# ashual/scene_generation

Hardware: AMD Instinct MI355X
Metric: images/sec G+D step, 128x128 <=8-obj scene graphs (higher is better)
Workload: dtype f32

## Files before the change

### scene_generation_amd/csrc/igemm_core.h

```cpp
#pragma once
#include <type_traits>
#include "common.h"
#include <stdlib.h>
#include <array>
#include <map>
#include <mutex>

typedef float f32x16 __attribute__((ext_vector_type(16)));


namespace sgk {
struct Gather {
  const float* src1; const float* src2;
  int C1, C2;
  int SH, SW;
  int LH, LW;
  int ushift;
  int PH, PW;
  int stride, sshift, pad, reflect;
  int bcast2;
  int pstep, ph0, pw0;
};

struct KEntry { unsigned choff; unsigned tapsel; };
// ... 3 lines not shown
extern thread_local double t_alg_bytes;
extern std::mutex g_tab_mu;
extern std::map<TabKey, TabEntry> g_tabs;
extern size_t g_tab_bytes;

int kn0_run(int KS, const float* A, int M, int K, const Gather& g, int NB, const float* bias, float* out, int Mtot, int act,
            float slope, double flops, void* ktab_ws, size_t ws_avail, hipStream_t s);
int kn1_run(int KS, const float* A, int M, int K, const Gather& g, int NB, const float* bias, float* out, int Mtot, int act,
            float slope, double flops, void* ktab_ws, size_t ws_avail, unsigned variant_stride, hipStream_t s);
int kn_sparse_run(int KS, const float* W, int M, int K, const Gather& g, int NB, const float* bias, float* out, int act,
                  float slope, const Sparse& sp, void* ws, hipStream_t s);
int kn_parity_run(int KS, const float* W, int Rdim, int B, int m0, int M, const Gather& g, int NB, const float* bias,
                  float* out, int Mtot, int act, float slope, double flops, void* ws, size_t ws_bytes, hipStream_t s);
int nk_run(int KS, const float* A, int M, int Mtot, const Gather& g, int NB, float* out, void* ws, size_t ws_bytes,
           double flops, hipStream_t s, const Sparse* sp, float* gb = nullptr, bool* gb_done = nullptr);
int skinny_vec(int align, int ld, int K);
int skinny_gemm(const float* a, int lda, int av, const float* b, int ldb, int bv, float* c, const float* bias,
                float* rowsum, int M, int N, int K, int act, float slope, hipStream_t s);
int skinny_gemm_gather(const float* obj, const float* pred, const int64_t* edges, int T, int Do, int Dp, const float* w, float* c,
                       const float* bias, int N, int act, float slope, hipStream_t s);
inline bool skinny_shape(int M, int N) {
  return (long)sg_cdiv(M, 32) * sg_cdiv(N, 32) <= (long)sg_opt(SG_OPT_LINEAR_SKINNY);
}
}

namespace {
using namespace sgk;
thread_local unsigned t_variant_stride = 0;

#ifdef SG_TIMELINE
__device__ unsigned long long* g_sg_tl = nullptr;
__device__ unsigned g_sg_tl_cap = 0;
#define SG_TL_STAMP(slot)                                                                       \
  do {                                                                                          \
    if (tl_on) tl_rec[slot] = __builtin_amdgcn_s_memtime();                                     \
  } while (0)
#else
#define SG_TL_STAMP(slot) do { } while (0)
#endif

#ifndef SG_NSUB
#define SG_NSUB 1
#endif
constexpr int BK = 16;

#ifndef SG_PIPE_DEFAULT
#define SG_PIPE_DEFAULT 2
#endif
template <int BM_, int BN_, int WGM_, int NSUB_, int PIPE_ = SG_PIPE_DEFAULT, int KFOLD_ = 0, int TS_ = (PIPE_ != 0 ? 1 : 0)>
struct TileCfg {
  static constexpr int BM = BM_, BN = BN_, WGM = WGM_, WGN = 4 / WGM_, NSUB = NSUB_, BKT = BK * NSUB_, PIPE = PIPE_;
  static constexpr int KFOLD = KFOLD_, TAILSPLIT = TS_;
  static_assert(TS_ == 0 || PIPE_ != 0, "tail split: pipelined loop only");
  static_assert(KFOLD_ == 0 || (PIPE_ != 0 && KFOLD_ % (BK * NSUB_) == 0), "KFOLD: whole k-tiles of the pipelined loop");
  static constexpr int WM = BM / WGM, WN = BN / WGN;
  static constexpr int TM = WM / 32, TN = WN / 32;
  static constexpr int LDA = BM + 4, LDB = BN + 4;
};

constexpr int LDK = BK + 4;



#ifndef SG_BUFLOAD
#define SG_BUFLOAD 1
#endif
constexpr int TAP_INVALID = SG_BUFLOAD ? (1 << 29) : -1;
#if SG_BUFLOAD
__device__ __forceinline__ __amdgpu_buffer_rsrc_t sg_rsrc(const float* p) {
  return __builtin_amdgcn_make_buffer_rsrc(const_cast<float*>(p), 0, 0x80000000u, 0x00020000);
}
__device__ __forceinline__ float sg_bufload(__amdgpu_buffer_rsrc_t r, unsigned elem) {
  return __builtin_bit_cast(float, __builtin_amdgcn_raw_buffer_load_b32(r, (int)(elem << 2), 0, 0));
}
__device__ __forceinline__ float4 sg_bufload4(__amdgpu_buffer_rsrc_t r, unsigned elem) {
  const auto v = __builtin_amdgcn_raw_buffer_load_b128(r, (int)(elem << 2), 0, 0);
  static_assert(sizeof(v) == 16, "raw_buffer_load_b128 must return 16 bytes");
  float4 f;
  __builtin_memcpy(&f, &v, 16);
  return f;
}
#endif
typedef unsigned int sg_u32x4 __attribute__((ext_vector_type(4)));
constexpr unsigned ELEM_INVALID = 1u << 29;
constexpr double SG_MAX_ELEMS = SG_BUFLOAD ? 536870912.0 : 2147483647.0;


template <int BX, bool VEC, bool MASK = true>
struct LoadKContig {
  const float* base; int ld; int X;
  static constexpr int LDS_INTS = 0;
  static constexpr int PASSES = BX >= 64 ? BX / 64 : 1;
  struct Stage { float r[PASSES * 4]; unsigned ok; };
  int x0_, xr_, kq_;
  unsigned voff_[PASSES];
  __device__ __forceinline__ void init(int x0, int tid, int*, int, int) {
    x0_ = x0; xr_ = tid >> 2; kq_ = (tid & 3) * 4;
#pragma unroll
    for (int p = 0; p < PASSES; ++p) {
      const int xl = xr_ + p * 64;
      const int x = x0_ + xl;
      const bool xok = (BX % 64 == 0 || xl < BX) && x < X;
      voff_[p] = xok ? ((unsigned)x * (unsigned)ld + (unsigned)kq_) * 4u : 0x80000000u;
    }
  }
  __device__ __forceinline__ void set_batch(int b, int stride, int) { base += (size_t)b * (size_t)stride; }
  __device__ __forceinline__ void prefetch(Stage&, int) const {}
  __device__ __forceinline__ void load(Stage& st, int k0, int kend) const {
    st.ok = 0;
#if SG_BUFLOAD
    if (VEC && (!MASK || k0 + BK <= kend)) {
      const __amdgpu_buffer_rsrc_t rs = sg_rsrc(base);
      const int so = __builtin_amdgcn_readfirstlane(k0 * 4);
#pragma unroll
      for (int p = 0; p < PASSES; ++p) {
        const auto v = __builtin_amdgcn_raw_buffer_load_b128(rs, (int)voff_[p], so, 0);
        __builtin_memcpy(&st.r[p * 4], &v, 16);
      }
      return;
    }
#endif
#pragma unroll
    for (int p = 0; p < PASSES; ++p) {
      const int xl = xr_ + p * 64;
      const int x = x0_ + xl, k = k0 + kq_;
      const bool xok = (BX % 64 == 0 || xl < BX) && x < X;
      const unsigned row = (unsigned)(xok ? x : 0) * (unsigned)ld;
      if (VEC && !MASK) {
        const float4 v = *reinterpret_cast<const float4*>(base + (unsigned)x * (unsigned)ld + k);
        st.r[p * 4 + 0] = v.x; st.r[p * 4 + 1] = v.y; st.r[p * 4 + 2] = v.z; st.r[p * 4 + 3] = v.w;
      } else if (VEC) {
        const bool ok = xok && k < kend;
#if SG_BUFLOAD
        const float4 v = sg_bufload4(sg_rsrc(base), ok ? row + (unsigned)k : ELEM_INVALID);
#else
        const float4 v = *reinterpret_cast<const float4*>(base + row + (ok ? k : 0));
        st.ok |= ok ? (15u << (p * 4)) : 0u;
#endif
        st.r[p * 4 + 0] = v.x; st.r[p * 4 + 1] = v.y; st.r[p * 4 + 2] = v.z; st.r[p * 4 + 3] = v.w;
      } else {
#pragma unroll
        for (int i = 0; i < 4; ++i) {
          const bool ok = xok && k + i < kend;
#if SG_BUFLOAD
          st.r[p * 4 + i] = sg_bufload(sg_rsrc(base), ok ? row + (unsigned)(k + i) : ELEM_INVALID);
#else
          st.r[p * 4 + i] = base[row + (ok ? k + i : 0)];
          st.ok |= ok ? (1u << (p * 4 + i)) : 0u;
#endif
        }
      }
    }
  }
  __device__ __forceinline__ void store(const Stage& st, float* T) const {
#pragma unroll
    for (int p = 0; p < PASSES; ++p) {
      const int xl = xr_ + p * 64;
      const bool in_tile = BX % 64 == 0 || xl < BX;
      if (in_tile && (SG_BUFLOAD || (VEC && !MASK))) {
        *reinterpret_cast<float4*>(T + xl * LDK + kq_) = make_float4(st.r[p * 4], st.r[p * 4 + 1], st.r[p * 4 + 2], st.r[p * 4 + 3]);
      } else if (in_tile) {
        float4 v;
        v.x = ((st.ok >> (p * 4 + 0)) & 1u) ? st.r[p * 4 + 0] : 0.f;
        v.y = ((st.ok >> (p * 4 + 1)) & 1u) ? st.r[p * 4 + 1] : 0.f;
        v.z = ((st.ok >> (p * 4 + 2)) & 1u) ? st.r[p * 4 + 2] : 0.f;
        v.w = ((st.ok >> (p * 4 + 3)) & 1u) ? st.r[p * 4 + 3] : 0.f;
// ... 90 lines not shown
  }
}


__global__ void build_ktab_kernel(KEntry* tab, int K, int Kpad, int KS2, int C1, int C2, unsigned shw, int bcast2,
                                  int tail_valid, unsigned variant_stride) {
  const int k = blockIdx.x * blockDim.x + threadIdx.x;
  if (k >= Kpad) return;
  KEntry e;
  if (k < K) {
    const int c = k / KS2, t = k - c * KS2;
    const bool second = C2 > 0 && c >= C1;
    const unsigned cc = (unsigned)(second ? c - C1 : c);
    e.choff = ((second && bcast2) ? cc : cc * shw) + (unsigned)t * variant_stride;
    e.tapsel = (unsigned)t | (second ? 256u : 0u);
  } else {
    e.choff = 0u; e.tapsel = tail_valid ? 0u : (unsigned)KS2;
  }
  tab[k] = e;
}

template <class Build>
const void* cached_table(TabKey key, size_t bytes, hipStream_t s, Build build) {
  int dev = 0;
  hipGetDevice(&dev);
  key[11] = dev;
  std::lock_guard<std::mutex> lk(g_tab_mu);
  auto it = g_tabs.find(key);
  if (it == g_tabs.end()) {
    TabEntry e{nullptr, bytes, nullptr, s};
    if (hipMalloc(&e.dev, bytes) != hipSuccess) return nullptr;
    hipEventCreateWithFlags(&e.ready, hipEventDisableTiming);
    build(e.dev);
    hipEventRecord(e.ready, s);
    g_tab_bytes += bytes;
    it = g_tabs.emplace(key, e).first;
  } else if (it->second.stream != s) {
    hipStreamCaptureStatus cs = hipStreamCaptureStatusNone;
    if (hipStreamIsCapturing(s, &cs) != hipSuccess || cs == hipStreamCaptureStatusNone) hipStreamWaitEvent(s, it->second.ready, 0);
  }
  return it->second.dev;
}

template <int BN, int KS, int MODE, bool TWO, bool MASK = true>
struct LoadGatherKN {
  Gather g; int Npix; const KEntry* ktab;
  static constexpr int KS2 = KS * KS;
  static constexpr int LDS_INTS = (KS2 + 1) * BN;
  static constexpr int ROWS = BN * BK / 256;
  static constexpr bool BUF = SG_BUFLOAD && MASK;
  struct Stage { float r[ROWS]; unsigned ok; KEntry e[ROWS]; };
  unsigned img1_, img2_, img2b_;
  int nl_, kr_;
  const int* tab_;
  __device__ __forceinline__ void set_batch(int b, int stride, int limit) { ktab += (size_t)b * (size_t)stride; Npix = limit; }
  __device__ __forceinline__ void init(int n0, int tid, int* tab, int, int) {
    nl_ = tid % BN;
    const int grp = tid / BN;
    kr_ = __builtin_amdgcn_readfirstlane(grp * ROWS);
    const int n = n0 + nl_;
    const bool okn = n < Npix;
    const int nn = okn ? n : 0;
    const int phw = g.PH * g.PW;
    const int img = nn / phw;
    const int pix = nn - img * phw;
    const int pi = pix / g.PW;
    const int ph = pi * g.pstep + g.ph0, pw = (pix - pi * g.PW) * g.pstep + g.pw0;
    int ah, aw;
    if (MODE == 0) { ah = ph * g.stride - g.pad; aw = pw * g.stride - g.pad; }
    else { ah = ph + g.pad; aw = pw + g.pad; }
    const unsigned shw = (unsigned)(g.SH * g.SW);
    img1_ = (unsigned)img * (unsigned)g.C1 * shw;
    img2_ = g.bcast2 ? (unsigned)img * (unsigned)g.C2 : (unsigned)img * (unsigned)g.C2 * shw;
    constexpr int G = 256 / BN;
    for (int t = grp; t <= KS2; t += G) {
      const int kh = t / KS, kw = t - kh * KS;
      int v = (okn && t < KS2) ? tap_offset<MODE>(g, ah, aw, kh, kw) : -1;
      if (BUF && v < 0) v = TAP_INVALID;
      tab[t * BN + nl_] = v;
    }
    tab_ = tab + nl_;
  }
  __device__ __forceinline__ void prefetch(Stage& st, int k0) const {
    const KEntry* e = ktab + (k0 + kr_);
#pragma unroll
    for (int i = 0; i < ROWS; ++i) st.e[i] = e[i];
  }
  __device__ __forceinline__ void load(Stage& st, int k0, int kend) const {
#if SG_BUFLOAD
    if (BUF) {
      const __amdgpu_buffer_rsrc_t r1 = sg_rsrc(g.src1);
#pragma unroll
      for (int i = 0; i < ROWS; ++i) {
        const unsigned choff = st.e[i].choff, ts = st.e[i].tapsel;
        const unsigned tp = (unsigned)tab_[(ts & 255u) * BN];
        if (TWO) {
          const bool second = (ts & 256u) != 0u;
          const unsigned t2 = (second && g.bcast2) ? (tp >= (unsigned)TAP_INVALID ? tp : 0u) : tp;
          st.r[i] = sg_bufload(second ? sg_rsrc(g.src2) : r1, (second ? img2_ : img1_) + choff + t2);
        } else {
          st.r[i] = sg_bufload(r1, img1_ + choff + tp);
        }
      }
      return;
    }
#endif
    st.ok = 0;
#pragma unroll
    for (int i = 0; i < ROWS; ++i) {
      const unsigned choff = st.e[i].choff, ts = st.e[i].tapsel;
      const int tp = tab_[(ts & 255u) * BN];
      const bool ok = !MASK || tp >= 0;
      if (TWO) {
        const bool second = (ts & 256u) != 0u;
        const float* base = second ? g.src2 : g.src1;
        const unsigned off = (second ? img2_ : img1_) + choff + ((second && g.bcast2) ? 0u : (unsigned)tp);
        st.r[i] = base[ok ? off : 0u];
      } else {
        st.r[i] = g.src1[ok ? img1_ + choff + (unsigned)tp : 0u];
      }
      st.ok |= ok ? (1u << i) : 0u;
    }
  }
  __device__ __forceinline__ void store(const Stage& st, float* T) const {
    if (BUF) store_krun<ROWS, false>(T, nl_, kr_, st.r, 0u);
    else store_krun<ROWS, MASK>(T, nl_, kr_, st.r, st.ok);
  }
};

struct FixedTaps { int lg; unsigned tapcode; };
template <int BN, int MODE>
struct LoadFixedKN {
  Gather g; int Npix; int KS; int lg; unsigned tapcode;
  int dedup;
  FastDiv dphw, dpw;
  static constexpr int LDS_INTS = 0;
  static constexpr int ROWS = BN * BK / 256;
  struct Stage { float r[ROWS]; };
  int nl_, kr_;
  unsigned voff_[ROWS];
  unsigned shw4_;
  __device__ __forceinline__ void set_batch(int, int, int) {}
  __device__ __forceinline__ void init(int n0, int tid, int*, int, int) {
    nl_ = tid % BN;
    kr_ = __builtin_amdgcn_readfirstlane((tid / BN) * ROWS);
    const int n = n0 + nl_;
    const bool okn = n < Npix;
    const int nn = okn ? n : 0;
    const int phw = g.PH * g.PW;
    const int img = (int)dphw.div((unsigned)nn);
    const int pix = nn - img * phw;
    const int pi = (int)dpw.div((unsigned)pix);
    const int ph = pi * g.pstep + g.ph0, pw = (pix - pi * g.PW) * g.pstep + g.pw0;
    int ah, aw;
    if (MODE == 0) { ah = ph * g.stride - g.pad; aw = pw * g.stride - g.pad; }
    else { ah = ph + g.pad; aw = pw + g.pad; }
    const unsigned shw = (unsigned)(g.SH * g.SW);
    shw4_ = shw * 4u;
    const unsigned img1 = (unsigned)img * (unsigned)g.C1 * shw;
    const int nt = 1 << lg;
    auto tap_voff = [&](int ti) -> unsigned {
      const int t = lg == 4 ? ti : (int)((tapcode >> (4 * ti)) & 15u);
      const int kh = KS == 4 ? (t >> 2) : (KS == 3 ? ((t * 11) >> 5) : (KS == 1 ? 0 : t / KS)), kw = t - kh * KS;
      const int v = okn ? tap_offset<MODE>(g, ah, aw, kh, kw) : -1;
      return v < 0 ? 0x80000000u : (img1 + (unsigned)v) * 4u;
    };
    if (lg <= 2 && dedup) {
      unsigned o[4];
      o[0] = tap_voff(0);
// ... 772 lines not shown
      for (int i = 0; i < TM; ++i) a[i] = *reinterpret_cast<const float4*>(A_ + i * 32 * LDK);
#pragma unroll
      for (int j = 0; j < TN; ++j) b[j] = *reinterpret_cast<const float4*>(B_ + j * 32 * LDK);
    };
    auto mma = [&](const float4 (&a)[TM], const float4 (&b)[TN]) {
#pragma unroll
      for (int e = 0; e < 4; ++e)
#pragma unroll
        for (int i = 0; i < TM; ++i)
#pragma unroll
          for (int j = 0; j < TN; ++j) {
            const float av = e == 0 ? a[i].x : (e == 1 ? a[i].y : (e == 2 ? a[i].z : a[i].w));
            const float bv = e == 0 ? b[j].x : (e == 1 ? b[j].y : (e == 2 ? b[j].z : b[j].w));
            acc[i][j] = __builtin_amdgcn_mfma_f32_32x32x2f32(av, bv, acc[i][j], 0, 0, 0);
          }
    };
    if (kbeg + BKT < kend) {
#pragma unroll
      for (int u = 0; u < NSUB; ++u) { al.load(sa[u], kbeg + BKT + u * BK, kend); bl.load(sb[u], kbeg + BKT + u * BK, kend); }
#pragma unroll
      for (int u = 0; u < NSUB; ++u) { al.prefetch(sa[u], kbeg + 2 * BKT + u * BK); bl.prefetch(sb[u], kbeg + 2 * BKT + u * BK); }
    }
    read_frag(0, 0, fa[0], fb[0]);
    if (AL::LDS_INTS > 0 || BL::LDS_INTS > 0) __syncthreads();
    constexpr bool FOLD = CFG::KFOLD > 0;
    f32x16 acc2[FOLD ? TM : 1][FOLD ? TN : 1];
    if constexpr (FOLD) {
#pragma unroll
      for (int i = 0; i < TM; ++i)
#pragma unroll
        for (int j = 0; j < TN; ++j)
#pragma unroll
          for (int r = 0; r < 16; ++r) acc2[i][j][r] = 0.f;
    }
    for (int k0 = kbeg; k0 < kend; k0 += BKT) {
      const bool more1 = k0 + BKT < kend, more2 = k0 + 2 * BKT < kend;
      if constexpr (FOLD) {
        if (k0 > kbeg && ((k0 - kbeg) % CFG::KFOLD) == 0) {
#pragma unroll
          for (int i = 0; i < TM; ++i)
#pragma unroll
            for (int j = 0; j < TN; ++j)
#pragma unroll
              for (int r = 0; r < 16; ++r) { acc2[i][j][r] += acc[i][j][r]; acc[i][j][r] = 0.f; }
        }
      }
      constexpr bool INTER = CFG::PIPE == 2 && 2 * NSUB <= 4;
      auto stage_next = [&]() {
        if (more2) {
#pragma unroll
          for (int u = 0; u < NSUB; ++u) { al.load(sa[u], k0 + 2 * BKT + u * BK, kend); bl.load(sb[u], k0 + 2 * BKT + u * BK, kend); }
#pragma unroll
          for (int u = 0; u < NSUB; ++u) { al.prefetch(sa[u], k0 + 3 * BKT + u * BK); bl.prefetch(sb[u], k0 + 3 * BKT + u * BK); }
        }
      };
      if (!INTER) {
        if (more1) {
#pragma unroll
          for (int u = 0; u < NSUB; ++u) { al.store(sa[u], As[buf ^ 1] + u * BM * LDK); bl.store(sb[u], Bs[buf ^ 1] + u * BN * LDK); }
        }
        stage_next();
      }
#pragma unroll
      for (int p = 0; p < P - 1; ++p) {
        read_frag(buf, p + 1, fa[(p + 1) & 1], fb[(p + 1) & 1]);
        __builtin_amdgcn_sched_barrier(0);
        if (INTER && p == 0) {
#pragma unroll
          for (int e = 0; e < 4; ++e) {
#pragma unroll
            for (int i = 0; i < TM; ++i)
#pragma unroll
              for (int j = 0; j < TN; ++j) {
                const float av = e == 0 ? fa[0][i].x : (e == 1 ? fa[0][i].y : (e == 2 ? fa[0][i].z : fa[0][i].w));
                const float bv = e == 0 ? fb[0][j].x : (e == 1 ? fb[0][j].y : (e == 2 ? fb[0][j].z : fb[0][j].w));
                acc[i][j] = __builtin_amdgcn_mfma_f32_32x32x2f32(av, bv, acc[i][j], 0, 0, 0);
              }
            __builtin_amdgcn_sched_barrier(0);
            if (more1 && e < 2 * NSUB) {
              const int u = e >> 1;
              if ((e & 1) == 0) al.store(sa[u], As[buf ^ 1] + u * BM * LDK);
              else bl.store(sb[u], Bs[buf ^ 1] + u * BN * LDK);
            }
            __builtin_amdgcn_sched_barrier(0);
          }
          stage_next();
        } else {
          mma(fa[p & 1], fb[p & 1]);
        }
        __builtin_amdgcn_sched_barrier(0);
      }
      __syncthreads();
      if (more1) read_frag(buf ^ 1, 0, fa[0], fb[0]);
      __builtin_amdgcn_sched_barrier(0);
      mma(fa[(P - 1) & 1], fb[(P - 1) & 1]);
      buf ^= 1;
    }
    if constexpr (FOLD) {
#pragma unroll
      for (int i = 0; i < TM; ++i)
#pragma unroll
        for (int j = 0; j < TN; ++j)
#pragma unroll
          for (int r = 0; r < 16; ++r) acc[i][j][r] = acc2[i][j][r] + acc[i][j][r];
    }
    SG_TL_STAMP(3);
    if (bi.prio) __builtin_amdgcn_s_setprio(3);
    if constexpr (TSPLIT) {
      if (ts_half >= 0) {
        int* ts_flag = reinterpret_cast<int*>(&As[0][0]);
        constexpr int PERW = TM * TN * 16 * 64;
        float* mine = bi.tail_slab + ((size_t)(ts_slot * ts_s + ts_half) * 4 + wid) * PERW;
        const __amdgpu_buffer_rsrc_t rm = __builtin_amdgcn_make_buffer_rsrc(mine, 0, PERW * 4, 0x00020000);
#pragma unroll
        for (int i = 0; i < TM; ++i)
#pragma unroll
          for (int j = 0; j < TN; ++j)
#pragma unroll
            for (int v = 0; v < 4; ++v) {
              sg_u32x4 d;
              __builtin_memcpy(&d, reinterpret_cast<const char*>(&acc[i][j]) + 16 * v, 16);
              __builtin_amdgcn_raw_buffer_store_b128(d, rm, (((i * TN + j) * 4 + v) * 64 + lane) * 16, 0, 16 );
            }
        if (!sg_arrive_last(bi.tail_cnt + ts_slot, ts_s, ts_flag)) return;
        const bool two = ts_s == 2;
        if (!two) {
#pragma unroll
          for (int i = 0; i < TM; ++i)
#pragma unroll
            for (int j = 0; j < TN; ++j)
#pragma unroll
              for (int r = 0; r < 16; ++r) acc[i][j][r] = 0.f;
        }
        for (int pc = 0; pc < ts_s; ++pc) {
          if (two && pc == ts_half) continue;
          const float* theirs = bi.tail_slab + ((size_t)(ts_slot * ts_s + pc) * 4 + wid) * PERW;
          const __amdgpu_buffer_rsrc_t rt = __builtin_amdgcn_make_buffer_rsrc(const_cast<float*>(theirs), 0, PERW * 4, 0x00020000);
#pragma unroll
          for (int i = 0; i < TM; ++i)
#pragma unroll
            for (int j = 0; j < TN; ++j)
#pragma unroll
              for (int v = 0; v < 4; ++v) {
                const auto d = __builtin_amdgcn_raw_buffer_load_b128(rt, (((i * TN + j) * 4 + v) * 64 + lane) * 16, 0, 16 );
                float4 f;
                __builtin_memcpy(&f, &d, 16);
                acc[i][j][4 * v + 0] += f.x; acc[i][j][4 * v + 1] += f.y; acc[i][j][4 * v + 2] += f.z; acc[i][j][4 * v + 3] += f.w;
              }
        }
      }
    }
    rowsum_finish(al, zblk);
    ep.store(acc, m0 + wm0, n0 + wn0, lane, zblk);
#ifdef SG_TIMELINE
    __builtin_amdgcn_s_waitcnt(0);
#endif
    SG_TL_STAMP(4);
    return;
  }
  for (int k0 = kbeg; k0 < kend; k0 += BKT) {
    const bool more = k0 + BKT < kend;
    if (more) {
#pragma unroll
      for (int u = 0; u < NSUB; ++u) { al.load(sa[u], k0 + BKT + u * BK, kend); bl.load(sb[u], k0 + BKT + u * BK, kend); }
#pragma unroll
      for (int u = 0; u < NSUB; ++u) { al.prefetch(sa[u], k0 + 2 * BKT + u * BK); bl.prefetch(sb[u], k0 + 2 * BKT + u * BK); }
// ... 636 lines not shown
```

### scene_generation_amd/csrc/norm.hip

```cpp
#include "common.h"
#include <stdlib.h>

namespace {

__device__ __forceinline__ float act_grad_from_pre(float pre, int act, float slope) {
  switch (act) {
    case SG_ACT_RELU: return pre > 0.f ? 1.f : 0.f;
    case SG_ACT_LEAKY: return pre > 0.f ? 1.f : slope;
    default: return 1.f;
  }
}

template <bool WAVE>
__global__ void __launch_bounds__(256) instnorm_fwd_kernel(const float* __restrict__ x, const float* __restrict__ skip,
                                                          float* __restrict__ y, float* __restrict__ mean_o,
                                                          float* __restrict__ rstd_o, int NC, int HW, float eps, int act,
                                                          float slope) {
  __shared__ float red[16];
  const int lane = threadIdx.x & 63;
  const int plane = WAVE ? blockIdx.x * 4 + (threadIdx.x >> 6) : blockIdx.x;
  if (WAVE && plane >= NC) return;
  const int t0 = WAVE ? lane : threadIdx.x, nt = WAVE ? 64 : blockDim.x;
  const float* xp = x + (size_t)plane * HW;
  float s = 0.f;
// ... 839 lines not shown
  const float* gp = gy + nc * OH * OW;
  float s = 0.f;
  for (int oh = ih / 2; oh <= (ih + 1) / 2; ++oh) {
    if (oh >= OH) continue;
    for (int ow = iw / 2; ow <= (iw + 1) / 2; ++ow) {
      if (ow >= OW) continue;
      s += gp[oh * OW + ow] / (float)(pool_cnt(oh, H) * pool_cnt(ow, W));
    }
  }
  gx[i] = s;
}

__device__ __forceinline__ int maxpool_argmax(float a, float b, float c, float d) {
  int k = 0; float m = a;
  if (b > m || b != b) { m = b; k = 1; }
  if (c > m || c != c) { m = c; k = 2; }
  if (d > m || d != d) { m = d; k = 3; }
  return k;
}
__global__ void maxpool2_fwd_kernel(const float* __restrict__ x, float* __restrict__ y, int NC, int H, int W, int OH, int OW) {
  const size_t i = (size_t)blockIdx.x * blockDim.x + threadIdx.x;
  if (i >= (size_t)NC * OH * OW) return;
  const int ow = i % OW;
  const int oh = (i / OW) % OH;
  const size_t nc = i / ((size_t)OW * OH);
  const float* p = x + (nc * H + 2 * oh) * W + 2 * ow;
  float a, b, c, d;
  if ((W & 1) == 0) {
    const float2 r0 = *reinterpret_cast<const float2*>(p), r1 = *reinterpret_cast<const float2*>(p + W);
    a = r0.x; b = r0.y; c = r1.x; d = r1.y;
  } else {
    a = p[0]; b = p[1]; c = p[W]; d = p[W + 1];
  }
  const int k = maxpool_argmax(a, b, c, d);
  y[i] = k == 0 ? a : (k == 1 ? b : (k == 2 ? c : d));
}
__global__ void maxpool2_bwd_kernel(const float* __restrict__ x, const float* __restrict__ gy, float* __restrict__ gx, int NC,
                                    int H, int W, int OH, int OW) {
  const int CW = (W + 1) / 2, CH = (H + 1) / 2;
  const size_t i = (size_t)blockIdx.x * blockDim.x + threadIdx.x;
  if (i >= (size_t)NC * CH * CW) return;
  const int cw = i % CW;
  const int ch = (i / CW) % CH;
  const size_t nc = i / ((size_t)CW * CH);
  const size_t base = (nc * H + 2 * ch) * W + 2 * cw;
  if (ch >= OH || cw >= OW) {
    for (int a = 0; a < 2; ++a)
      for (int b = 0; b < 2; ++b)
        if (2 * ch + a < H && 2 * cw + b < W) gx[base + a * W + b] = 0.f;
    return;
  }
  const float* p = x + base;
  const float g = gy[(nc * OH + ch) * OW + cw];
  const int k = maxpool_argmax(p[0], p[1], p[W], p[W + 1]);
  if ((W & 1) == 0) {
    *reinterpret_cast<float2*>(gx + base) = make_float2(k == 0 ? g : 0.f, k == 1 ? g : 0.f);
    *reinterpret_cast<float2*>(gx + base + W) = make_float2(k == 2 ? g : 0.f, k == 3 ? g : 0.f);
  } else {
    gx[base] = k == 0 ? g : 0.f; gx[base + 1] = k == 1 ? g : 0.f;
    gx[base + W] = k == 2 ? g : 0.f; gx[base + W + 1] = k == 3 ? g : 0.f;
  }
}

__global__ void gap_fwd_kernel(const float* __restrict__ x, float* __restrict__ y, int NC, int HW) {
  const int plane = blockIdx.x * 4 + (threadIdx.x >> 6), lane = threadIdx.x & 63;
  if (plane >= NC) return;
  const float* xp = x + (size_t)plane * HW;
  float s = 0.f;
  for (int i = lane; i < HW; i += 64) s += xp[i];
  s = sg_wave_sum(s);
  if (lane == 0) y[plane] = s / (float)HW;
}

__global__ void gap_bwd_kernel(const float* __restrict__ gy, float* __restrict__ gx, size_t total, int HW) {
  const size_t i = (size_t)blockIdx.x * blockDim.x + threadIdx.x;
  if (i < total) gx[i] = gy[i / HW] / (float)HW;
}

__global__ void act_fwd_kernel(const float* __restrict__ x, float* __restrict__ y, size_t n, int act, float slope) {
  const size_t i = (size_t)blockIdx.x * blockDim.x + threadIdx.x;
  if (i < n) y[i] = sg_apply_act(x[i], act, slope);
}

__global__ void act_bwd_kernel(const float* __restrict__ y, const float* __restrict__ gy, float* __restrict__ gx, size_t n,
                               int act, float slope) {
  const size_t i = (size_t)blockIdx.x * blockDim.x + threadIdx.x;
  if (i >= n) return;
  const float o = y[i];
  float d = 1.f;
  switch (act) {
    case SG_ACT_RELU: d = o > 0.f ? 1.f : 0.f; break;
    case SG_ACT_LEAKY: d = o > 0.f ? 1.f : slope; break;
    case SG_ACT_TANH: d = 1.f - o * o; break;
    case SG_ACT_SIGMOID: d = o * (1.f - o); break;
    default: break;
  }
  gx[i] = gy[i] * d;
}

__global__ void upsample2_fwd_kernel(const float* __restrict__ x, float* __restrict__ y, size_t total, int H, int W) {
  const size_t i = (size_t)blockIdx.x * blockDim.x + threadIdx.x;
  if (i >= total) return;
  const int ow = i % (2 * W);
  const int oh = (i / (2 * W)) % (2 * H);
  const size_t nc = i / ((size_t)4 * W * H);
  y[i] = x[nc * H * W + (size_t)(oh >> 1) * W + (ow >> 1)];
}

__global__ void reflect_pad_fwd_kernel(const float* __restrict__ x, float* __restrict__ y, size_t total, int H, int W,
                                       int pad) {
  const size_t i = (size_t)blockIdx.x * blockDim.x + threadIdx.x;
  if (i >= total) return;
  const int PW = W + 2 * pad, PH = H + 2 * pad;
  const int ow = i % PW;
  const int oh = (i / PW) % PH;
  const size_t nc = i / ((size_t)PW * PH);
  int ih = oh - pad, iw = ow - pad;
  ih = ih < 0 ? -ih : (ih >= H ? 2 * H - 2 - ih : ih);
  iw = iw < 0 ? -iw : (iw >= W ? 2 * W - 2 - iw : iw);
  y[i] = x[nc * H * W + (size_t)ih * W + iw];
}

__device__ __forceinline__ int reflect_sources(int l, int L, int p, int (&a)[3]) {
  int n = 0;
  a[n++] = l + p;
  if (l >= 1 && l <= p) a[n++] = p - l;
  if (l <= L - 2 && l >= L - 1 - p) a[n++] = p + 2 * L - 2 - l;
  return n;
}

__global__ void pad_upsample_bwd_kernel(const float* __restrict__ gp, float* __restrict__ gx, int H, int W, int pad, int ups) {
  const unsigned j = blockIdx.x * blockDim.x + threadIdx.x;
  if (j >= (unsigned)(H * W)) return;
  const size_t nc = blockIdx.y;
  const int h = (int)(j / (unsigned)W), w = (int)(j - (unsigned)h * (unsigned)W);
  const int LH = H * ups, LW = W * ups, PH = LH + 2 * pad, PW = LW + 2 * pad;
  const float* g = gp + nc * PH * PW;
  float s = 0.f;
  for (int dh = 0; dh < ups; ++dh) {
    int ah[3];
    const int nh = reflect_sources(h * ups + dh, LH, pad, ah);
    for (int dw = 0; dw < ups; ++dw) {
      int aw[3];
      const int nw = reflect_sources(w * ups + dw, LW, pad, aw);
      for (int a = 0; a < nh; ++a)
        for (int b = 0; b < nw; ++b) s += g[ah[a] * PW + aw[b]];
    }
  }
  gx[nc * H * W + j] = s;
}

struct FoldPlan {
  int hq0, hq1, wq0, wq1, iblocks;
  FastDiv dnq, dW, dWb;
};
__global__ void __launch_bounds__(256) reflect_fold_kernel(const float* __restrict__ gp, float* __restrict__ gx, int H, int W,
                                                           int pad, FoldPlan fp) {
  const size_t nc = blockIdx.y;
  const int PW = W + 2 * pad, PH = H + 2 * pad;
  const float* g = gp + nc * PH * PW;
  float* o = gx + nc * H * W;
  const int rows = fp.hq1 - fp.hq0, nq = (fp.wq1 - fp.wq0) >> 2;
  if ((int)blockIdx.x < fp.iblocks) {
    const unsigned id = blockIdx.x * 256u + threadIdx.x;
    if (id >= (unsigned)(rows * nq)) return;
    const unsigned r = fp.dnq.div(id), q = id - r * (unsigned)nq;
    const int h = fp.hq0 + (int)r, w0 = fp.wq0 + 4 * (int)q;
    const float* src = g + (unsigned)((h + pad) * PW + pad + w0);
    float* dst = o + (unsigned)(h * W + w0);
    float4 v;
    if ((reinterpret_cast<uintptr_t>(src) & 15) == 0) v = *reinterpret_cast<const float4*>(src);
    else v = make_float4(src[0], src[1], src[2], src[3]);
    v = make_float4(0.f + v.x, 0.f + v.y, 0.f + v.z, 0.f + v.w);
    if ((reinterpret_cast<uintptr_t>(dst) & 15) == 0) *reinterpret_cast<float4*>(dst) = v;
    else { dst[0] = v.x; dst[1] = v.y; dst[2] = v.z; dst[3] = v.w; }
    return;
  }
  const unsigned id = (blockIdx.x - (unsigned)fp.iblocks) * 256u + threadIdx.x;
  const int Wb = W - 4 * nq, ntb = (H - rows) * W;
  if (id >= (unsigned)(ntb + rows * Wb)) return;
// ... 303 lines not shown
  hipLaunchKernelGGL(bn_bwd_stats_kernel, dim3(C, S), dim3(256), 0, s, x, gy, gamma, beta, save_mean, save_rstd, part, N, C,
                     HW, S, act, slope, counter, sums, ggamma, gbeta);
  if (!counter)
    hipLaunchKernelGGL(bn_bwd_final_kernel, dim3(sg_cdiv(C, 64)), dim3(64), 0, s, (const float*)part, sums, ggamma, gbeta, C, S);
  if (bn_apply_per_plane(HW))
    hipLaunchKernelGGL(bn_bwd_apply_kernel, dim3(sg_cdiv(HW, 1024), N * C), dim3(256), 0, s, x, gy, gamma, beta, save_mean,
                       save_rstd, (const float*)sums, gx, C, HW, 1.f / ((float)N * HW), training, act, slope);
  else
    hipLaunchKernelGGL(bn_bwd_apply_flat_kernel, dim3(sg_cdiv((size_t)N * C * HW, 256)), dim3(256), 0, s, x, gy, gamma, beta,
                       save_mean, save_rstd, (const float*)sums, gx, (size_t)N * C * HW, C, HW, 1.f / ((float)N * HW),
                       training, act, slope);
  SG_LAUNCH_CHECK("sg_batchnorm_bwd");
  return 0;
}
extern "C" size_t sg_channel_sum_ws_bytes(int C) { return (size_t)C * 64 * sizeof(float); }

extern "C" int sg_channel_sum(const float* g, float* out, int N, int C, int HW, void* ws, size_t ws_bytes,
                              sgStream stream) {
  SG_ARG_CHECK(g && out && N > 0 && C > 0 && HW > 0, "sg_channel_sum: bad arguments");
  hipStream_t s = (hipStream_t)stream;
  const int S = channel_sum_slices(N, C, HW, ws ? ws_bytes : 0);
  if (S <= 1) {
    hipLaunchKernelGGL(channel_sum_kernel, dim3(C), dim3(256), 0, s, g, out, N, C, HW);
  } else {
    float* part = reinterpret_cast<float*>(ws);
    int* counter = C <= 4096 ? sg_counter_alloc(s, C, false, 4) : nullptr;
    hipLaunchKernelGGL(channel_sum_partial_kernel, dim3(C, S), dim3(256), 0, s, g, part, N, C, HW, S, counter, out);
    if (!counter)
      hipLaunchKernelGGL(channel_sum_final_kernel, dim3(sg_cdiv(C, 64)), dim3(64), 0, s, (const float*)part, out, C, S);
  }
  SG_LAUNCH_CHECK("sg_channel_sum");
  return 0;
}

extern "C" int sg_avgpool3s2_fwd(const float* x, float* y, int NC, int H, int W, int OH, int OW, sgStream stream) {
  SG_ARG_CHECK(x && y && OH == (H + 2 - 3) / 2 + 1 && OW == (W + 2 - 3) / 2 + 1, "sg_avgpool3s2_fwd: bad arguments");
  hipLaunchKernelGGL(avgpool3s2_fwd_kernel, grid1d((size_t)NC * OH * OW), dim3(256), 0, (hipStream_t)stream, x, y, NC, H, W, OH, OW);
  SG_LAUNCH_CHECK("sg_avgpool3s2_fwd");
  return 0;
}

extern "C" int sg_avgpool3s2_bwd(const float* gy, float* gx, int NC, int H, int W, int OH, int OW, sgStream stream) {
  SG_ARG_CHECK(gy && gx, "sg_avgpool3s2_bwd: bad arguments");
  hipLaunchKernelGGL(avgpool3s2_bwd_kernel, grid1d((size_t)NC * H * W), dim3(256), 0, (hipStream_t)stream, gy, gx, NC, H, W, OH, OW);
  SG_LAUNCH_CHECK("sg_avgpool3s2_bwd");
  return 0;
}

extern "C" int sg_maxpool2_fwd(const float* x, float* y, int NC, int H, int W, sgStream stream) {
  SG_ARG_CHECK(x && y && NC > 0 && H >= 2 && W >= 2, "sg_maxpool2_fwd: bad arguments");
  const int OH = H / 2, OW = W / 2;
  SG_ARG_CHECK((double)NC * H * W < 2147483647.0 * 2, "sg_maxpool2_fwd: tensor too large");
  hipLaunchKernelGGL(maxpool2_fwd_kernel, grid1d((size_t)NC * OH * OW), dim3(256), 0, (hipStream_t)stream, x, y, NC, H, W, OH, OW);
  SG_LAUNCH_CHECK("sg_maxpool2_fwd");
  return 0;
}

extern "C" int sg_maxpool2_bwd(const float* x, const float* gy, float* gx, int NC, int H, int W, sgStream stream) {
  SG_ARG_CHECK(x && gy && gx && NC > 0 && H >= 2 && W >= 2, "sg_maxpool2_bwd: bad arguments");
  const int OH = H / 2, OW = W / 2;
  hipLaunchKernelGGL(maxpool2_bwd_kernel, grid1d((size_t)NC * ((H + 1) / 2) * ((W + 1) / 2)), dim3(256), 0, (hipStream_t)stream,
                     x, gy, gx, NC, H, W, OH, OW);
  SG_LAUNCH_CHECK("sg_maxpool2_bwd");
  return 0;
}

extern "C" int sg_gap_fwd(const float* x, float* y, int NC, int HW, sgStream stream) {
  SG_ARG_CHECK(x && y && NC > 0 && HW > 0, "sg_gap_fwd: bad arguments");
  hipLaunchKernelGGL(gap_fwd_kernel, dim3(sg_cdiv(NC, 4)), dim3(256), 0, (hipStream_t)stream, x, y, NC, HW);
  SG_LAUNCH_CHECK("sg_gap_fwd");
  return 0;
}

extern "C" int sg_gap_bwd(const float* gy, float* gx, int NC, int HW, sgStream stream) {
  SG_ARG_CHECK(gy && gx && NC > 0 && HW > 0, "sg_gap_bwd: bad arguments");
  hipLaunchKernelGGL(gap_bwd_kernel, grid1d((size_t)NC * HW), dim3(256), 0, (hipStream_t)stream, gy, gx, (size_t)NC * HW, HW);
  SG_LAUNCH_CHECK("sg_gap_bwd");
  return 0;
}

extern "C" int sg_act_fwd(const float* x, float* y, int64_t n, int act, float slope, sgStream stream) {
  SG_ARG_CHECK(x && y && n >= 0, "sg_act_fwd: bad arguments");
  if (n == 0) return 0;
  hipLaunchKernelGGL(act_fwd_kernel, grid1d((size_t)n), dim3(256), 0, (hipStream_t)stream, x, y, (size_t)n, act, slope);
  SG_LAUNCH_CHECK("sg_act_fwd");
  return 0;
}

extern "C" int sg_act_bwd(const float* y, const float* gy, float* gx, int64_t n, int act, float slope, sgStream stream) {
  SG_ARG_CHECK(y && gy && gx && n >= 0, "sg_act_bwd: bad arguments");
  if (n == 0) return 0;
  hipLaunchKernelGGL(act_bwd_kernel, grid1d((size_t)n), dim3(256), 0, (hipStream_t)stream, y, gy, gx, (size_t)n, act, slope);
  SG_LAUNCH_CHECK("sg_act_bwd");
  return 0;
}

extern "C" int sg_upsample2_fwd(const float* x, float* y, int NC, int H, int W, sgStream stream) {
  SG_ARG_CHECK(x && y, "sg_upsample2_fwd: bad arguments");
  const size_t total = (size_t)NC * 4 * H * W;
  hipLaunchKernelGGL(upsample2_fwd_kernel, grid1d(total), dim3(256), 0, (hipStream_t)stream, x, y, total, H, W);
  SG_LAUNCH_CHECK("sg_upsample2_fwd");
  return 0;
}

extern "C" int sg_reflect_pad_fwd(const float* x, float* y, int NC, int H, int W, int pad, sgStream stream) {
  SG_ARG_CHECK(x && y && pad < H && pad < W, "sg_reflect_pad_fwd: bad arguments");
  const size_t total = (size_t)NC * (H + 2 * pad) * (W + 2 * pad);
  hipLaunchKernelGGL(reflect_pad_fwd_kernel, grid1d(total), dim3(256), 0, (hipStream_t)stream, x, y, total, H, W, pad);
  SG_LAUNCH_CHECK("sg_reflect_pad_fwd");
  return 0;
}

extern "C" int sg_pool2d_fwd(const float* x, float* y, int NC, int H, int W, int k, int avg, sgStream stream) {
  SG_ARG_CHECK(x && y && NC > 0 && k >= 1 && H >= k && W >= k, "sg_pool2d_fwd: bad arguments");
  const int OH = H / k, OW = W / k;
  const size_t total = (size_t)NC * OH * OW;
  hipLaunchKernelGGL(pool2d_fwd_kernel, grid1d(total), dim3(256), 0, (hipStream_t)stream, x, y, total, H, W, OH, OW, k, avg);
  SG_LAUNCH_CHECK("sg_pool2d_fwd");
  return 0;
}

extern "C" int sg_pool2d_bwd(const float* x, const float* gy, float* gx, int NC, int H, int W, int k, int avg, sgStream stream) {
  SG_ARG_CHECK((x || avg) && gy && gx && NC > 0 && k >= 1 && H >= k && W >= k, "sg_pool2d_bwd: bad arguments");
  const size_t total = (size_t)NC * H * W;
  hipLaunchKernelGGL(pool2d_bwd_kernel, grid1d(total), dim3(256), 0, (hipStream_t)stream, x, gy, gx, total, H, W, H / k, W / k, k, avg);
  SG_LAUNCH_CHECK("sg_pool2d_bwd");
  return 0;
}

extern "C" int sg_replicate_pad_fwd(const float* x, float* y, int NC, int H, int W, int pad, sgStream stream) {
  SG_ARG_CHECK(x && y && NC > 0 && H > 0 && W > 0 && pad >= 0, "sg_replicate_pad_fwd: bad arguments");
  const size_t total = (size_t)NC * (H + 2 * pad) * (W + 2 * pad);
  hipLaunchKernelGGL(replicate_pad_fwd_kernel, grid1d(total), dim3(256), 0, (hipStream_t)stream, x, y, total, H, W, pad);
  SG_LAUNCH_CHECK("sg_replicate_pad_fwd");
  return 0;
}

extern "C" int sg_replicate_pad_bwd(const float* gp, float* gx, int NC, int H, int W, int pad, sgStream stream) {
  SG_ARG_CHECK(gp && gx && NC > 0 && H > 0 && W > 0 && pad >= 0, "sg_replicate_pad_bwd: bad arguments");
  const size_t total = (size_t)NC * H * W;
  hipLaunchKernelGGL(replicate_pad_bwd_kernel, grid1d(total), dim3(256), 0, (hipStream_t)stream, gp, gx, total, H, W, pad);
  SG_LAUNCH_CHECK("sg_replicate_pad_bwd");
  return 0;
}

extern "C" int sg_pad_upsample_bwd(const float* gp, float* gx, int NC, int H, int W, int pad, int upsample,
                                   sgStream stream) {
  SG_ARG_CHECK(gp && gx && (upsample == 1 || upsample == 2) && pad >= 0, "sg_pad_upsample_bwd: bad arguments");
  if (NC == 0 || H * W == 0) return 0;
  for (int n0 = 0; n0 < NC; n0 += 65535) {
    const int nn = NC - n0 < 65535 ? NC - n0 : 65535;
    const size_t PP = (size_t)(H * upsample + 2 * pad) * (W * upsample + 2 * pad);
    if (upsample == 1) {
      FoldPlan fp;
      fp.hq0 = pad + 1; fp.hq1 = H - 1 - pad; fp.wq0 = (pad + 1 + 3) & ~3; fp.wq1 = (W - 1 - pad) & ~3;
      if (fp.hq1 <= fp.hq0 || fp.wq1 <= fp.wq0) { fp.hq0 = fp.hq1 = 0; fp.wq0 = fp.wq1 = 0; }
      const int rows = fp.hq1 - fp.hq0, nq = (fp.wq1 - fp.wq0) / 4, Wb = W - 4 * nq;
      fp.iblocks = sg_cdiv(rows * nq, 256);
      fp.dnq = FastDiv((unsigned)(nq > 0 ? nq : 1)); fp.dW = FastDiv((unsigned)W); fp.dWb = FastDiv((unsigned)(Wb > 0 ? Wb : 1));
      const int ring = (H - rows) * W + rows * Wb;
      hipLaunchKernelGGL(reflect_fold_kernel, dim3(fp.iblocks + sg_cdiv(ring, 256), nn), dim3(256), 0, (hipStream_t)stream,
                         gp + (size_t)n0 * PP, gx + (size_t)n0 * H * W, H, W, pad, fp);
      continue;
    }
    hipLaunchKernelGGL(pad_upsample_bwd_kernel, dim3(sg_cdiv(H * W, 256), nn), dim3(256), 0, (hipStream_t)stream,
                       gp + (size_t)n0 * PP, gx + (size_t)n0 * H * W, H, W, pad, upsample);
  }
  SG_LAUNCH_CHECK("sg_pad_upsample_bwd");
  return 0;
}

extern "C" int sg_concat_channels(const float* a, const float* b, float* out, int N, int Ca, int Cb, int HW,
                                  sgStream stream) {
  SG_ARG_CHECK(a && b && out, "sg_concat_channels: bad arguments");
  const size_t total = (size_t)N * (Ca + Cb) * HW;
// ... 47 lines not shown
```

Baseline: 1132.

## Vectorize activation kernels, load k-table via constant address space, add vmcnt wait

Activation forward and backward kernels gain float4 variants, used when the element count is a multiple of four and the pointers are 16-byte aligned, so fewer, wider memory accesses are issued. In the implicit-GEMM gather loader, the per-k table entries are now read through an address_space(4) (constant) pointer so the compiler can use scalar loads. An explicit s_waitcnt vmcnt(0) is inserted after the last interleaved LDS store in the MFMA loop, which may stall earlier than the compiler would but makes the ordering explicit. These are unrelated micro-optimizations across two files.

```diff
diff --git a/scene_generation_amd/csrc/igemm_core.h b/scene_generation_amd/csrc/igemm_core.h
--- a/scene_generation_amd/csrc/igemm_core.h
+++ b/scene_generation_amd/csrc/igemm_core.h
@@ -109,6 +109,7 @@
 }
 #endif
 typedef unsigned int sg_u32x4 __attribute__((ext_vector_type(4)));
+__device__ __forceinline__ void sg_wait_vm0() { __builtin_amdgcn_s_waitcnt(0x0F70); }
 constexpr unsigned ELEM_INVALID = 1u << 29;
 constexpr double SG_MAX_ELEMS = SG_BUFLOAD ? 536870912.0 : 2147483647.0;
 
@@ -365,9 +366,10 @@
     tab_ = tab + nl_;
   }
   __device__ __forceinline__ void prefetch(Stage& st, int k0) const {
-    const KEntry* e = ktab + (k0 + kr_);
-#pragma unroll
-    for (int i = 0; i < ROWS; ++i) st.e[i] = e[i];
+    typedef const KEntry __attribute__((address_space(4))) * ConstKEntryPtr;
+    const ConstKEntryPtr e = (ConstKEntryPtr)(ktab + (k0 + kr_));
+#pragma unroll
+    for (int i = 0; i < ROWS; ++i) { st.e[i].choff = e[i].choff; st.e[i].tapsel = e[i].tapsel; }
   }
   __device__ __forceinline__ void load(Stage& st, int k0, int kend) const {
 #if SG_BUFLOAD
@@ -1306,6 +1308,7 @@
               if ((e & 1) == 0) al.store(sa[u], As[buf ^ 1] + u * BM * LDK);
               else bl.store(sb[u], Bs[buf ^ 1] + u * BN * LDK);
             }
+            if (e == 2 * NSUB - 1) sg_wait_vm0();
             __builtin_amdgcn_sched_barrier(0);
           }
           stage_next();
diff --git a/scene_generation_amd/csrc/norm.hip b/scene_generation_amd/csrc/norm.hip
--- a/scene_generation_amd/csrc/norm.hip
+++ b/scene_generation_amd/csrc/norm.hip
@@ -945,11 +945,7 @@
   if (i < n) y[i] = sg_apply_act(x[i], act, slope);
 }
 
-__global__ void act_bwd_kernel(const float* __restrict__ y, const float* __restrict__ gy, float* __restrict__ gx, size_t n,
-                               int act, float slope) {
-  const size_t i = (size_t)blockIdx.x * blockDim.x + threadIdx.x;
-  if (i >= n) return;
-  const float o = y[i];
+__device__ __forceinline__ float act_deriv(float o, int act, float slope) {
   float d = 1.f;
   switch (act) {
     case SG_ACT_RELU: d = o > 0.f ? 1.f : 0.f; break;
@@ -958,7 +954,35 @@
     case SG_ACT_SIGMOID: d = o * (1.f - o); break;
     default: break;
   }
-  gx[i] = gy[i] * d;
+  return d;
+}
+
+__global__ void act_bwd_kernel(const float* __restrict__ y, const float* __restrict__ gy, float* __restrict__ gx, size_t n,
+                               int act, float slope) {
+  const size_t i = (size_t)blockIdx.x * blockDim.x + threadIdx.x;
+  if (i >= n) return;
+  gx[i] = gy[i] * act_deriv(y[i], act, slope);
+}
+
+__global__ void act_fwd_vec_kernel(const float4* __restrict__ x, float4* __restrict__ y, size_t n4, int act, float slope) {
+  const size_t i = (size_t)blockIdx.x * blockDim.x + threadIdx.x;
+  if (i >= n4) return;
+  const float4 v = x[i];
+  y[i] = make_float4(sg_apply_act(v.x, act, slope), sg_apply_act(v.y, act, slope), sg_apply_act(v.z, act, slope),
+                     sg_apply_act(v.w, act, slope));
+}
+
+__global__ void act_bwd_vec_kernel(const float4* __restrict__ y, const float4* __restrict__ gy, float4* __restrict__ gx, size_t n4,
+                                   int act, float slope) {
+  const size_t i = (size_t)blockIdx.x * blockDim.x + threadIdx.x;
+  if (i >= n4) return;
+  const float4 o = y[i], g = gy[i];
+  gx[i] = make_float4(g.x * act_deriv(o.x, act, slope), g.y * act_deriv(o.y, act, slope), g.z * act_deriv(o.z, act, slope),
+                      g.w * act_deriv(o.w, act, slope));
+}
+
+inline bool act_vec_ok(int64_t n, const void* a, const void* b, const void* c) {
+  return n % 4 == 0 && ((reinterpret_cast<uintptr_t>(a) | reinterpret_cast<uintptr_t>(b) | reinterpret_cast<uintptr_t>(c)) & 15) == 0;
 }
 
 __global__ void upsample2_fwd_kernel(const float* __restrict__ x, float* __restrict__ y, size_t total, int H, int W) {
@@ -1428,7 +1452,11 @@
 extern "C" int sg_act_fwd(const float* x, float* y, int64_t n, int act, float slope, sgStream stream) {
   SG_ARG_CHECK(x && y && n >= 0, "sg_act_fwd: bad arguments");
   if (n == 0) return 0;
-  hipLaunchKernelGGL(act_fwd_kernel, grid1d((size_t)n), dim3(256), 0, (hipStream_t)stream, x, y, (size_t)n, act, slope);
+  if (act_vec_ok(n, x, y, y))
+    hipLaunchKernelGGL(act_fwd_vec_kernel, grid1d((size_t)n / 4), dim3(256), 0, (hipStream_t)stream, (const float4*)x, (float4*)y,
+                       (size_t)n / 4, act, slope);
+  else
+    hipLaunchKernelGGL(act_fwd_kernel, grid1d((size_t)n), dim3(256), 0, (hipStream_t)stream, x, y, (size_t)n, act, slope);
   SG_LAUNCH_CHECK("sg_act_fwd");
   return 0;
 }
@@ -1436,7 +1464,11 @@
 extern "C" int sg_act_bwd(const float* y, const float* gy, float* gx, int64_t n, int act, float slope, sgStream stream) {
   SG_ARG_CHECK(y && gy && gx && n >= 0, "sg_act_bwd: bad arguments");
   if (n == 0) return 0;
-  hipLaunchKernelGGL(act_bwd_kernel, grid1d((size_t)n), dim3(256), 0, (hipStream_t)stream, y, gy, gx, (size_t)n, act, slope);
+  if (act_vec_ok(n, y, gy, gx))
+    hipLaunchKernelGGL(act_bwd_vec_kernel, grid1d((size_t)n / 4), dim3(256), 0, (hipStream_t)stream, (const float4*)y,
+                       (const float4*)gy, (float4*)gx, (size_t)n / 4, act, slope);
+  else
+    hipLaunchKernelGGL(act_bwd_kernel, grid1d((size_t)n), dim3(256), 0, (hipStream_t)stream, y, gy, gx, (size_t)n, act, slope);
   SG_LAUNCH_CHECK("sg_act_bwd");
   return 0;
 }
```

Result: no change. 1143, median of 6 (+1.0%).
